# microsoft/ptgnn

Hardware: NVIDIA H100
Metric: edges/sec per GNN layer (higher is better)
Workload: dtype f32

## Files before the change

ptgnn_b200/csrc/fused_mp.cu:

```cuda
#include "fused_mp.cuh"

#include <cuda_bf16.h>
#include <cuda_fp16.h>
#include <float.h>
#include <stdlib.h>

#include <type_traits>

#include "tc_common.cuh"

namespace ptgnn {
namespace fused {

using tc::mbar_arrive;
using tc::mbar_init;
using tc::mbar_wait;

constexpr int NUM_THREADS = 12 * 32;
constexpr int GATHER_WARP0 = 8, GATHER_THREADS = 64;
constexpr int SCHED_WARP = 10;
constexpr int NUM_CONSUMER_WARPS = 8 + 2;
constexpr int NUM_SLOTS = 3, LOOKAHEAD = 2;
constexpr int SLOT_BYTES = 32768;
constexpr int RING_BYTES = NUM_SLOTS * SLOT_BYTES;
constexpr int META_RING = 8;
constexpr int SCHED_RING = 4;
constexpr int CONSUMER_REGS = 224, PRODUCER_REGS = 56;
static_assert(PRODUCER_REGS + 2 * CONSUMER_REGS <= 3 * 168, "register budgets exceed the launch allocation");
constexpr int NMAX = 64;
constexpr int ACC_PITCH = NMAX + 4;
constexpr int ACC_BYTES = kD * ACC_PITCH * 4;
constexpr int ALL_BAR_ID = 1, GRP_BAR_ID = 2;

struct Meta {
    int32_t tloff[128];
    uint32_t endmask[4];
    uint32_t lowmask[4];
    int32_t n, pad[3];
};
struct Sched {
    int32_t blk, pad[3];
    int32_t off[PTGNN_MAX_EDGE_TYPES + 4];
};
constexpr int ACC_OFF = RING_BYTES;
constexpr int AGG_OFF = RING_BYTES + ACC_BYTES;
__host__ __device__ constexpr int agg_bytes(int B) { return B * kD * 4; }
constexpr int SMEM_TAIL = META_RING * (int)sizeof(Meta) + SCHED_RING * (int)sizeof(Sched) + 256 ;
constexpr int smem_bytes(int B) { return 1024 + RING_BYTES + ACC_BYTES + agg_bytes(B) + SMEM_TAIL; }
static_assert(smem_bytes(kMaxBlockTargets) <= 232448, "shared memory budget");

struct Params {
    const unsigned char *src_rows, *tgt_rows;
    const uint4 *wpack;
    const int32_t *group_off, *src_f;
    const uint8_t *tl_f;
    const int32_t *row_ptr;
    void *out;
    int num_nodes, num_blocks, B, T, reduce, out_mode;
    int32_t *status;
    unsigned long long *trace;
    Epilogue epi;
};

__device__ __forceinline__ uint4 ldg_nc_u4(const uint4 *p) {
    uint4 r;
    asm volatile("ld.global.nc.L1::no_allocate.v4.u32 {%0,%1,%2,%3}, [%4];" : "=r"(r.x), "=r"(r.y), "=r"(r.z), "=r"(r.w) : "l"(p));
    return r;
}
__device__ __forceinline__ void named_bar_sync(int id, int threads) { asm volatile("bar.sync %0, %1;" ::"r"(id), "r"(threads) : "memory"); }
__device__ __forceinline__ uint32_t swz(int row, int q) { return (uint32_t)(row * 128 + ((q ^ (row & 7)) << 4)); }

constexpr int TRACE_ROLES = 3, TRACE_CAP = 8192;
__shared__ uint32_t trace_n[TRACE_ROLES];
__device__ __forceinline__ void trace_mark(const Params &p, int tag, uint32_t step) {
    if (p.trace == nullptr || blockIdx.x != 0) return;
    const int tid = (int)threadIdx.x;
    const int role = tid == GATHER_WARP0 * 32 ? 0 : (tid == 0 ? 1 : (tid == 128 ? 2 : -1));
    if (role < 0) return;
    const uint32_t n = trace_n[role];
    if (n >= TRACE_CAP) return;
    p.trace[role * TRACE_CAP + n] = ((unsigned long long)clock64() << 24) | ((unsigned long long)(step & 0xFFFFu) << 8) | (unsigned)(tag & 0xFF);
    trace_n[role] = n + 1;
}

struct Step { int blk, t, e, n, seg; bool first_sub, last_sub; };
template <int NSEG>
struct StepGen {
    const Sched *sched;
    uint64_t *sfull, *sempty;
    int T, nmax, lane;
    uint32_t it = 0;
    const Sched *tab = nullptr;
    int blk = -1, t = 0, e0 = 0, e = 0, e1 = 0, seg = 0;
    bool in_block = false;
    __device__ __forceinline__ int next(Step &s) {
        for (;;) {
            if (!in_block) {
                const uint32_t r = it % SCHED_RING;
                mbar_wait(&sfull[r], (it / SCHED_RING) & 1);
                tab = &sched[r];
                blk = tab->blk;
                if (blk < 0) return 2;
                in_block = true;
                t = -1; e = e1 = 0; seg = 0;
            }
            if (e < e1) {
                s.blk = blk; s.t = t; s.e = e; s.n = min(nmax, e1 - e); s.seg = seg;
                s.first_sub = e == e0; s.last_sub = e + nmax >= e1;
                if (++seg == NSEG) { seg = 0; e += nmax; }
                return 0;
            }
            ++t;
            while (t < T && tab->off[t + 1] == tab->off[t]) ++t;
            if (t >= T) {
                in_block = false;
                s.blk = blk;
                __syncwarp();
                if (lane == 0) mbar_arrive(&sempty[it % SCHED_RING]);
                ++it;
                return 1;
            }
            e0 = e = tab->off[t]; e1 = tab->off[t + 1]; seg = 0;
        }
    }
};

template <int RED>
__device__ __forceinline__ void continue_segment(float &t, float prev, float v, uint32_t start_bit) {
    if (RED == PTGNN_REDUCE_MAX)
        asm("{\n\t.reg .pred pc;\n\tsetp.eq.u32 pc, %3, 0;\n\t@pc max.f32 %0, %1, %2;\n\t}" : "+f"(t) : "f"(prev), "f"(v), "r"(start_bit));
    else if (RED == PTGNN_REDUCE_MIN)
        asm("{\n\t.reg .pred pc;\n\tsetp.eq.u32 pc, %3, 0;\n\t@pc min.f32 %0, %1, %2;\n\t}" : "+f"(t) : "f"(prev), "f"(v), "r"(start_bit));
    else
        asm("{\n\t.reg .pred pc;\n\tsetp.eq.u32 pc, %3, 0;\n\t@pc add.f32 %0, %1, %2;\n\t}" : "+f"(t) : "f"(prev), "f"(v), "r"(start_bit));
}
__device__ __forceinline__ void sts_f32_if(uint32_t addr, float v, uint32_t bit) {
    asm volatile("{\n\t.reg .pred pe;\n\tsetp.ne.u32 pe, %2, 0;\n\t@pe st.shared.f32 [%0], %1;\n\t}" ::"r"(addr), "f"(v), "r"(bit) : "memory");
}
__device__ __forceinline__ float4 lds_f32x4(uint32_t addr) {
    float4 v;
    asm volatile("ld.shared.v4.f32 {%0, %1, %2, %3}, [%4];" : "=f"(v.x), "=f"(v.y), "=f"(v.z), "=f"(v.w) : "r"(addr));
    return v;
}
__device__ __forceinline__ void sts_f32x4(uint32_t addr, float4 v) {
    asm volatile("st.shared.v4.f32 [%0], {%1, %2, %3, %4};" ::"r"(addr), "f"(v.x), "f"(v.y), "f"(v.z), "f"(v.w) : "memory");
}
__device__ __forceinline__ float lds_f32(uint32_t addr) {
    float v;
    asm volatile("ld.shared.f32 %0, [%1];" : "=f"(v) : "r"(addr) : "memory");
    return v;
}

__device__ __forceinline__ uint32_t pack_h2(__half a, __half b) {
    return (uint32_t)__half_as_ushort(a) | ((uint32_t)__half_as_ushort(b) << 16);
}
__device__ __forceinline__ bool split_f16(float x, __half &hi, __half &lo) {
    hi = __float2half_rn(x);
    lo = __float2half_rn((x - __half2float(hi)) * 2048.0f);
    return fabsf(x) < 65504.0f;
}

template <int RED> __device__ __forceinline__ float red_identity() {
    return RED == PTGNN_REDUCE_MAX ? -FLT_MAX : (RED == PTGNN_REDUCE_MIN ? FLT_MAX : 0.0f);
}
template <int RED> __device__ __forceinline__ float red_op(float a, float m) {
    if (RED == PTGNN_REDUCE_MAX) return fmaxf(a, m);
    if (RED == PTGNN_REDUCE_MIN) return fminf(a, m);
    return a + m;
}

template <int RED, bool WHOLE_ROW>
__device__ __forceinline__ void write_out_block(const Params *p, uint32_t agg_saddr, int row0, int row_lo, int row_hi, int r_first,
                                                int r_step, int q) {
    const float IDENT = red_identity<RED>();
    const int rows = min(p->B, p->num_nodes - row0);
    const int my_hi = min(row_hi, rows);
    const float4 ident4 = make_float4(IDENT, IDENT, IDENT, IDENT);
    auto finish_row = [&](auto mode_tag, auto plain_tag, int r, float4 a) {
        constexpr int MODE = decltype(mode_tag)::value;
        constexpr bool PLAIN = decltype(plain_tag)::value;
        const int v = row0 + r;
        if (!PLAIN) {
            if (RED == PTGNN_REDUCE_MEAN) {
                const int cnt = __ldg(p->row_ptr + v + 1) - __ldg(p->row_ptr + v);
                const float c = (float)(cnt < 1 ? 1 : cnt);
                a.x /= c; a.y /= c; a.z /= c; a.w /= c;
            }
            if (RED == PTGNN_REDUCE_MAX || RED == PTGNN_REDUCE_MIN) {
                if (a.x == IDENT) a.x = 0.0f;
                if (a.y == IDENT) a.y = 0.0f;
                if (a.z == IDENT) a.z = 0.0f;
                if (a.w == IDENT) a.w = 0.0f;
            }
            if (p->epi.act != PTGNN_ACT_NONE) {
                a.x = apply_act(a.x, p->epi.act); a.y = apply_act(a.y, p->epi.act);
                a.z = apply_act(a.z, p->epi.act); a.w = apply_act(a.w, p->epi.act);
            }
            if (WHOLE_ROW && p->epi.ln_w != nullptr) {
                float sum = (a.x + a.y) + (a.z + a.w);
#pragma unroll
                for (int o = 16; o > 0; o >>= 1) sum += __shfl_xor_sync(0xffffffffu, sum, o);
                const float mean = sum / (float)kD;
                const float dx = a.x - mean, dy = a.y - mean, dz = a.z - mean, dw = a.w - mean;
                float qq = (dx * dx + dy * dy) + (dz * dz + dw * dw);
#pragma unroll
                for (int o = 16; o > 0; o >>= 1) qq += __shfl_xor_sync(0xffffffffu, qq, o);
                const float rstd = rsqrtf(qq / (float)kD + p->epi.ln_eps);
                const float4 w = *reinterpret_cast<const float4 *>(p->epi.ln_w + q * 4);
                const float4 b = *reinterpret_cast<const float4 *>(p->epi.ln_b + q * 4);
                a.x = dx * rstd * w.x + b.x; a.y = dy * rstd * w.y + b.y;
                a.z = dz * rstd * w.z + b.z; a.w = dw * rstd * w.w + b.w;
            }
        }
        if (MODE == 1) {
            __nv_bfloat162 lo = __floats2bfloat162_rn(a.x, a.y), hi = __floats2bfloat162_rn(a.z, a.w);
            uint2 pk;
            pk.x = *reinterpret_cast<uint32_t *>(&lo); pk.y = *reinterpret_cast<uint32_t *>(&hi);
            reinterpret_cast<uint2 *>(p->out)[(size_t)v * (kD / 4) + q] = pk;
        } else if (MODE == 2) {
            const __half2 h01 = __floats2half2_rn(a.x, a.y), h23 = __floats2half2_rn(a.z, a.w);
            const float2 f01 = __half22float2(h01), f23 = __half22float2(h23);
            const __half2 l01 = __floats2half2_rn((a.x - f01.x) * 2048.0f, (a.y - f01.y) * 2048.0f);
            const __half2 l23 = __floats2half2_rn((a.z - f23.x) * 2048.0f, (a.w - f23.y) * 2048.0f);
            uint2 *row = reinterpret_cast<uint2 *>(p->out) + (size_t)v * (2 * kD / 4);
            row[q] = make_uint2(*reinterpret_cast<const uint32_t *>(&h01), *reinterpret_cast<const uint32_t *>(&h23));
            row[kD / 4 + q] = make_uint2(*reinterpret_cast<const uint32_t *>(&l01), *reinterpret_cast<const uint32_t *>(&l23));
            const float big = fmaxf(fmaxf(fabsf(a.x), fabsf(a.y)), fmaxf(fabsf(a.z), fabsf(a.w)));
            if (!(big < 65504.0f) && p->status != nullptr) *reinterpret_cast<volatile int32_t *>(p->status) = 1;
        } else {
            reinterpret_cast<float4 *>(p->out)[(size_t)v * (kD / 4) + q] = a;
        }
    };
    auto write_rows = [&](auto mode_tag, auto plain_tag) {
        for (int r0 = row_lo + r_first; r0 < my_hi; r0 += 2 * r_step) {
            float4 v4[2];
#pragma unroll
            for (int u = 0; u < 2; ++u) {
                const int r = r0 + r_step * u;
                if (r < my_hi) {
                    const uint32_t rowa = agg_saddr + (uint32_t)(r * kD + q * 4) * 4u;
                    v4[u] = lds_f32x4(rowa);
                    sts_f32x4(rowa, ident4);
                }
            }
#pragma unroll
            for (int u = 0; u < 2; ++u)
                if (r0 + r_step * u < my_hi) finish_row(mode_tag, plain_tag, r0 + r_step * u, v4[u]);
        }
    };
    const bool plain = RED == PTGNN_REDUCE_SUM && p->epi.act == PTGNN_ACT_NONE && p->epi.ln_w == nullptr;
    using std::integral_constant;
    if (p->out_mode == 2) { if (plain) write_rows(integral_constant<int, 2>{}, integral_constant<bool, true>{}); else write_rows(integral_constant<int, 2>{}, integral_constant<bool, false>{}); }
    else if (p->out_mode == 1) { if (plain) write_rows(integral_constant<int, 1>{}, integral_constant<bool, true>{}); else write_rows(integral_constant<int, 1>{}, integral_constant<bool, false>{}); }
    else { if (plain) write_rows(integral_constant<int, 0>{}, integral_constant<bool, true>{}); else write_rows(integral_constant<int, 0>{}, integral_constant<bool, false>{}); }
}

template <int NPROD, int K, int NSEG, int RED>
__global__ void __launch_bounds__(NUM_THREADS, 1) fused_aggregate_kernel(const __grid_constant__ Params p) {
    constexpr int NPART = NPROD == 3 ? 2 : 1;
    constexpr int ROW_BYTES = K * 2 * NPART;
    constexpr int KCH = K / 64;
    constexpr int NT = NPART * KCH;
    constexpr int TILE_BYTES = NMAX * 128;
    static_assert(NT * TILE_BYTES <= SLOT_BYTES, "slot size");
    constexpr bool BF16 = NPROD == 1;

    extern __shared__ unsigned char smem_raw[];
    unsigned char *ring = smem_raw + ((1024u - (smem_u32(smem_raw) & 1023u)) & 1023u);
    float *acc_s = reinterpret_cast<float *>(ring + ACC_OFF);
    float *agg_s = reinterpret_cast<float *>(ring + AGG_OFF);
    unsigned char *tail = ring + AGG_OFF + agg_bytes(p.B);
    Meta *meta_ring = reinterpret_cast<Meta *>(tail);
    Sched *sched = reinterpret_cast<Sched *>(tail + META_RING * sizeof(Meta));
    uint64_t *bars = reinterpret_cast<uint64_t *>(tail + META_RING * sizeof(Meta) + SCHED_RING * sizeof(Sched));
    uint64_t *x_full = bars, *x_empty = bars + 3, *sched_full = bars + 6, *sched_empty = bars + 10;

    const int warp = __shfl_sync(0xffffffffu, (int)(threadIdx.x >> 5), 0);
    const int lane = threadIdx.x & 31;
    if (threadIdx.x == 0) {
        for (int s = 0; s < NUM_SLOTS; ++s) { mbar_init(&x_full[s], 2 * GATHER_THREADS); mbar_init(&x_empty[s], 8); }
        for (int r = 0; r < SCHED_RING; ++r) { mbar_init(&sched_full[r], 1); mbar_init(&sched_empty[r], NUM_CONSUMER_WARPS); }
        for (int r = 0; r < TRACE_ROLES; ++r) trace_n[r] = 0;
        tc::mbar_init_fence();
    }
    __syncthreads();
    const int T = p.T;

    if (warp >= GATHER_WARP0) {
        tc::reg_dealloc<PRODUCER_REGS>();
        if (warp == SCHED_WARP) {
            for (uint32_t i = 0;; ++i) {
                const uint32_t r = i % SCHED_RING;
                mbar_wait(&sched_empty[r], ((i / SCHED_RING) & 1) ^ 1);
                const long long blk = (long long)blockIdx.x + (long long)i * gridDim.x;
                const bool valid = blk < p.num_blocks;
                Sched *e = &sched[r];
                if (valid) {
                    for (int t = lane; t <= T; t += 32) e->off[t] = __ldg(p.group_off + blk * T + t);
                }
                if (lane == 0) e->blk = valid ? (int)blk : -1;
                __syncwarp();
                if (lane == 0) mbar_arrive(&sched_full[r]);
                if (!valid) break;
            }
        } else if (warp < GATHER_WARP0 + GATHER_THREADS / 32) {
            const int g = (int)threadIdx.x - GATHER_WARP0 * 32;
            const int q = g & 7, rsub = g >> 3;
            StepGen<NSEG> gen{sched, sched_full, sched_empty, T, NMAX, lane};
            uint32_t c_issue = 0, c_done = 0, sgc = 0;
            Step cur, nxt;
            bool has_nxt = false;
            int idx_nxt[NMAX / 8];
            int tl_a[NMAX / 64], tl_b[NMAX / 64];
            auto fetch = [&]() {
                int ev;
                do { ev = gen.next(nxt); } while (ev == 1);
                has_nxt = ev == 0;
                if (!has_nxt) return;
                if (nxt.seg == 0) {
#pragma unroll
                    for (int i = 0; i < NMAX / 8; ++i) {
                        const int r = rsub + 8 * i;
                        idx_nxt[i] = r < nxt.n ? __ldg(p.src_f + nxt.e + r) : -1;
                    }
#pragma unroll
                    for (int half = 0; half < NMAX / 64; ++half) {
                        const int c = g + 64 * half;
                        tl_a[half] = c < nxt.n ? (int)__ldg(p.tl_f + nxt.e + c) : -1;
                        tl_b[half] = c + 1 < nxt.n ? (int)__ldg(p.tl_f + nxt.e + c + 1) : -2;
                    }
                } else {
#pragma unroll
                    for (int i = 0; i < NMAX / 8; ++i) {
                        const int r = rsub + 8 * i;
                        idx_nxt[i] = r < nxt.n ? nxt.blk * p.B + (int)__ldg(p.tl_f + nxt.e + r) : -1;
                    }
                }
            };
            auto finish_meta = [&](const Step &st) {
                if (st.seg != 0) return;
                Meta *m = &meta_ring[sgc % META_RING];
#pragma unroll
                for (int half = 0; half < NMAX / 64; ++half) {
                    const int c = g + 64 * half;
                    const bool valid = tl_a[half] >= 0;
                    const bool end = valid && tl_b[half] != tl_a[half];
                    m->tloff[c] = valid ? tl_a[half] * (kD * 4) : 0;
                    const uint32_t word = __ballot_sync(0xffffffffu, end);
                    const uint32_t low = __ballot_sync(0xffffffffu, valid && tl_a[half] < (p.B >> 1));
                    if (lane == 0) { m->endmask[c >> 5] = word; m->lowmask[c >> 5] = low; }
                }
                if (g == 0) m->n = st.n;
                ++sgc;
            };
            auto issue_next = [&]() {
                cur = nxt;
                int idx[NMAX / 8];
#pragma unroll
                for (int i = 0; i < NMAX / 8; ++i) idx[i] = idx_nxt[i];
                finish_meta(cur);
                const uint32_t slot = c_issue % NUM_SLOTS;
                trace_mark(p, 1, c_issue);
                mbar_wait(&x_empty[slot], ((c_issue / NUM_SLOTS) & 1) ^ 1);
                trace_mark(p, 2, c_issue);
                const unsigned char *rows = cur.seg == 0 ? p.src_rows : p.tgt_rows;
                const uint32_t sbase = smem_u32(ring + slot * SLOT_BYTES) + swz(rsub, q);
#pragma unroll
                for (int i = 0; i < NMAX / 8; ++i) {
                    if (idx[i] >= 0) {
                        const unsigned char *src = rows + (size_t)idx[i] * ROW_BYTES + q * 16;
#pragma unroll
                        for (int ti = 0; ti < NT; ++ti)
                            cp_async16(sbase + ti * TILE_BYTES + i * 1024, src + (ti / KCH) * (K * 2) + (ti % KCH) * 128, 16);
                    }
                }
                trace_mark(p, 3, c_issue);
                ++c_issue;
            };
            fetch();
            bool more = has_nxt;
            while (more) {
                const uint32_t slot = c_issue % NUM_SLOTS;
                issue_next();
                asm volatile("cp.async.mbarrier.arrive.noinc.shared::cta.b64 [%0];" ::"r"(smem_u32(&x_full[slot])) : "memory");
                trace_mark(p, 4, c_done);
                mbar_arrive(&x_full[slot]);
                ++c_done;
                fetch();
                more = has_nxt;
            }
            cp_async_wait<0>();
        }
    } else {
        tc::reg_alloc<CONSUMER_REGS>();
        constexpr bool SPLIT = NPROD == 3;
        const int eg = warp >> 2, ew = warp & 3;
        const int d = ew * 32 + lane;
        const int gq = lane >> 2, tq = lane & 3;
        const int f0 = 64 * eg + 16 * ew + gq;
        const int fw = SPLIT ? 64 * eg + (d & 63) : d, half = SPLIT ? d >> 6 : eg;
        const uint32_t aggcol_s = smem_u32(agg_s + fw);
        const uint32_t accrow_s = smem_u32(acc_s + fw * ACC_PITCH);
        const int grp_bar = GRP_BAR_ID + eg;
        const int stage_bar = SPLIT ? grp_bar : ALL_BAR_ID, stage_threads = SPLIT ? 128 : 256;
        const float IDENT = red_identity<RED>();
        StepGen<NSEG> gen{sched, sched_full, sched_empty, T, NMAX, lane};
        {
            const int row_lo = half == 0 ? 0 : (p.B >> 1), row_hi = half == 0 ? (p.B >> 1) : p.B;
            for (int r = row_lo; r < row_hi; ++r) agg_s[r * kD + fw] = IDENT;
        }
        uint32_t sg = 0, xs = 0;
        int w_t = -1, w_seg = -1;
        uint32_t wf[NPART][K / 16][4];
        float acc_m[32], acc_c[32];
        float acc = IDENT;
        auto load_weights = [&](const Step &st) {
            const uint32_t *wp = reinterpret_cast<const uint32_t *>(p.wpack + (size_t)(st.t * NSEG + st.seg) * NPART * (K / 8) * 128);
#pragma unroll
            for (int part = 0; part < NPART; ++part)
#pragma unroll
                for (int ks = 0; ks < K / 16; ++ks)
#pragma unroll
                    for (int i = 0; i < 4; ++i) {
                        const int c4 = (part * (K / 8) + 2 * ks + (i >> 1)), f = f0 + 8 * (i & 1);
                        wf[part][ks][i] = __ldg(wp + ((size_t)c4 * 128 + f) * 4 + tq);
                    }
            w_t = st.t; w_seg = st.seg;
            trace_mark(p, 11, xs);
        };
        auto mma = [&](auto nb_tag, uint32_t slot_addr) {
            constexpr int NB = decltype(nb_tag)::value;
#pragma unroll
            for (int ks = 0; ks < K / 16; ++ks) {
                const int kc = ks >> 2, kk = ks & 3;
                const uint64_t x_hi = tc::make_smem_desc_sw128(slot_addr + kc * TILE_BYTES) + kk * 2;
                const uint64_t x_lo = tc::make_smem_desc_sw128(slot_addr + (KCH + kc) * TILE_BYTES) + kk * 2;
                auto one = [&](float (&dacc)[32], const uint32_t (&a)[4], uint64_t desc) {
                    if (NB == 1) tc::wgmma_16_rs_n16<BF16>(dacc, a, desc);
                    else if (NB == 2) tc::wgmma_16_rs_n32<BF16>(dacc, a, desc);
                    else if (NB == 3) tc::wgmma_16_rs_n48<BF16>(dacc, a, desc);
                    else tc::wgmma_16_rs_n64<BF16>(dacc, a, desc);
                };
                one(acc_m, wf[0][ks], x_hi);
                if (NPROD == 3) {
                    one(acc_c, wf[0][ks], x_lo);
                    one(acc_c, wf[NPART - 1][ks], x_hi);
                }
            }
        };
        Step s, nx;
        int ev = gen.next(s);
        while (ev != 2) {
            if (ev == 0) {
                trace_mark(p, 10, xs);
                if (s.t != w_t || s.seg != w_seg) load_weights(s);
                const uint32_t slot = xs % NUM_SLOTS;
                mbar_wait(&x_full[slot], (xs / NUM_SLOTS) & 1);
                tc::fence_proxy_async_smem();
                trace_mark(p, 12, xs);
                if (tc::warp_uniform(s.seg) == 0) {
#pragma unroll
                    for (int i = 0; i < 32; ++i) { acc_m[i] = 0.0f; acc_c[i] = 0.0f; }
                }
                const uint32_t slot_addr = smem_u32(ring + slot * SLOT_BYTES);
                const int nb = tc::warp_uniform((s.n + 15) >> 4);
                tc::wgmma_fence();
                using std::integral_constant;
                if (nb == 1) mma(integral_constant<int, 1>{}, slot_addr);
                else if (nb == 2) mma(integral_constant<int, 2>{}, slot_addr);
                else if (nb == 3) mma(integral_constant<int, 3>{}, slot_addr);
                else mma(integral_constant<int, 4>{}, slot_addr);
                tc::wgmma_commit();
                trace_mark(p, 13, xs);
                tc::wgmma_wait<0>();
                tc::fence_acc(acc_m);
                tc::fence_acc(acc_c);
                __syncwarp();
                if (lane == 0) mbar_arrive(&x_empty[slot]);
                trace_mark(p, 14, xs);
                ++xs;
                const int evn = gen.next(nx);
                if (SPLIT && evn == 0 && (nx.t != w_t || nx.seg != w_seg)) load_weights(nx);
                if (s.seg == NSEG - 1) {
                    trace_mark(p, 20, sg);
                    named_bar_sync(stage_bar, stage_threads);
#pragma unroll
                    for (int j = 0; j < 8; ++j) {
                        if (8 * j < 16 * nb) {
#pragma unroll
                        for (int h = 0; h < 2; ++h) {
                            float v0 = acc_m[4 * j + 2 * h], v1 = acc_m[4 * j + 2 * h + 1];
                            if (NPROD == 3) { v0 = fmaf(acc_c[4 * j + 2 * h], 1.0f / 2048.0f, v0); v1 = fmaf(acc_c[4 * j + 2 * h + 1], 1.0f / 2048.0f, v1); }
                            *reinterpret_cast<float2 *>(acc_s + (f0 + 8 * h) * ACC_PITCH + 8 * j + 2 * tq) = make_float2(v0, v1);
                        }
                        }
                    }
                    named_bar_sync(stage_bar, stage_threads);
                    trace_mark(p, 21, sg);
                    const Meta *m = &meta_ring[sg % META_RING];
                    const int n = s.n;
                    int split = __popc(m->lowmask[0]) + __popc(m->lowmask[1]);
                    const int c_lo = half == 0 ? 0 : split, c_hi = half == 0 ? split : n;
                    constexpr int W = 16;
                    for (int c0 = c_lo & ~15; c0 < c_hi; c0 += 16) {
                        uint32_t vm[W];
#pragma unroll
                        for (int j = 0; j < W / 4; ++j) {
                            const float4 v4 = lds_f32x4(accrow_s + (uint32_t)(c0 + 4 * j) * 4u);
                            vm[4 * j] = __float_as_uint(v4.x); vm[4 * j + 1] = __float_as_uint(v4.y);
                            vm[4 * j + 2] = __float_as_uint(v4.z); vm[4 * j + 3] = __float_as_uint(v4.w);
                        }
                        uint32_t addr[W];
#pragma unroll
                        for (int j = 0; j < W / 4; ++j) {
                            const int4 o = *reinterpret_cast<const int4 *>(&m->tloff[c0 + 4 * j]);
                            addr[4 * j] = aggcol_s + o.x; addr[4 * j + 1] = aggcol_s + o.y;
                            addr[4 * j + 2] = aggcol_s + o.z; addr[4 * j + 3] = aggcol_s + o.w;
                        }
                        const uint32_t endw = (m->endmask[c0 >> 5] >> (c0 & 31)) & 0xFFFFu;
                        const uint32_t prev_end = c0 == 0 ? 1u : (m->endmask[(c0 - 1) >> 5] >> ((c0 - 1) & 31)) & 1u;
                        const uint32_t startw = (endw << 1) | prev_end;
                        const int first = c_lo > c0 ? c_lo - c0 : 0, last = c_hi - c0 < W ? c_hi - c0 : W;
                        const uint32_t storew = endw & (0xFFFFu << first) & (0xFFFFu >> (W - last));
                        float pre[W];
#pragma unroll
                        for (int c = 0; c < W; ++c) pre[c] = lds_f32(addr[c]);
                        float t[W];
                        constexpr bool ADD = RED == PTGNN_REDUCE_SUM || RED == PTGNN_REDUCE_MEAN;
#pragma unroll
                        for (int c = 0; c < W; ++c) {
                            float v = __uint_as_float(vm[c]);
                            if (NPROD == 1) {
                                v = __bfloat162float(__float2bfloat16_rn(v));
                                vm[c] = __float_as_uint(v);
                            }
                            t[c] = ADD ? __fadd_rn(pre[c], v) : red_op<RED>(pre[c], v);
                        }
                        continue_segment<RED>(t[0], acc, __uint_as_float(vm[0]), startw & 1u);
#pragma unroll
                        for (int c = 1; c < W; ++c) continue_segment<RED>(t[c], t[c - 1], __uint_as_float(vm[c]), startw & (1u << c));
                        acc = t[W - 1];
#pragma unroll
                        for (int c = 0; c < W; ++c) sts_f32_if(addr[c], t[c], storew & (1u << c));
                    }
                    trace_mark(p, 22, sg);
                    ++sg;
                }
                s = nx; ev = evn;
                continue;
            }
            const int blk = s.blk;
            const int evn = gen.next(nx);
            if (SPLIT && evn == 0 && (nx.t != w_t || nx.seg != w_seg)) load_weights(nx);
            trace_mark(p, 23, sg);
            if (SPLIT && p.epi.ln_w == nullptr) {
                named_bar_sync(grp_bar, 128);
                write_out_block<RED, false>(&p, smem_u32(agg_s), blk * p.B, 0, p.B, 2 * ew + (lane >> 4), 8, 16 * eg + (lane & 15));
            } else {
                const int wbar = SPLIT ? ALL_BAR_ID : grp_bar, wthreads = SPLIT ? 256 : 128;
                named_bar_sync(wbar, wthreads);
                const int row_lo = eg == 0 ? 0 : (p.B >> 1), row_hi = eg == 0 ? (p.B >> 1) : p.B;
                write_out_block<RED, true>(&p, smem_u32(agg_s), blk * p.B, row_lo, row_hi, ew, 4, lane);
                named_bar_sync(wbar, wthreads);
            }
            trace_mark(p, 24, sg);
            s = nx; ev = evn;
        }
    }
}

__global__ void __launch_bounds__(256) pack_states_kernel(const float *__restrict__ h, long long rows, int K,
                                                          uint4 *__restrict__ out, int32_t *__restrict__ status) {
    const long long total = rows * (K / 8);
    bool bad = false;
    for (long long i = (long long)blockIdx.x * blockDim.x + threadIdx.x; i < total; i += (long long)gridDim.x * blockDim.x) {
        const long long row = i / (K / 8);
        const int c8 = (int)(i - row * (K / 8));
        const float4 a = ld_stream_f4(reinterpret_cast<const float4 *>(h + row * K + c8 * 8));
        const float4 b = ld_stream_f4(reinterpret_cast<const float4 *>(h + row * K + c8 * 8 + 4));
        const float x[8] = {a.x, a.y, a.z, a.w, b.x, b.y, b.z, b.w};
        __half hi[8], lo[8];
#pragma unroll
        for (int j = 0; j < 8; ++j) bad |= !split_f16(x[j], hi[j], lo[j]);
        uint4 vh, vl;
        vh.x = pack_h2(hi[0], hi[1]); vh.y = pack_h2(hi[2], hi[3]); vh.z = pack_h2(hi[4], hi[5]); vh.w = pack_h2(hi[6], hi[7]);
        vl.x = pack_h2(lo[0], lo[1]); vl.y = pack_h2(lo[2], lo[3]); vl.z = pack_h2(lo[4], lo[5]); vl.w = pack_h2(lo[6], lo[7]);
        uint4 *dst = out + row * (K / 4);
        dst[c8] = vh;
        dst[K / 8 + c8] = vl;
    }
    if (bad && status != nullptr) *reinterpret_cast<volatile int32_t *>(status) = 1;
}

struct WeightSrc {
    const float *w[PTGNN_MAX_EDGE_TYPES];
};
template <int NPROD>
__global__ void __launch_bounds__(256) pack_weights_kernel(const __grid_constant__ WeightSrc src, int num_types, int K, int nseg,
                                                           uint4 *__restrict__ out, int32_t *__restrict__ status) {
    constexpr int NPART = NPROD == 3 ? 2 : 1;
    const int per_mat = nseg * (K / 8) * 128;
    const long long total = (long long)num_types * per_mat;
    bool bad = false;
    for (long long i = (long long)blockIdx.x * blockDim.x + threadIdx.x; i < total; i += (long long)gridDim.x * blockDim.x) {
        const int t = (int)(i / per_mat);
        int r = (int)(i - (long long)t * per_mat);
        const int seg = r / ((K / 8) * 128);
        r -= seg * (K / 8) * 128;
        const int c4 = r / 128, d = r % 128;
        const float *row = src.w[t] + (size_t)d * (nseg * K) + seg * K + c4 * 8;
        float x[8];
#pragma unroll
        for (int j = 0; j < 8; ++j) x[j] = row[j];
        const size_t base = ((size_t)(t * nseg + seg) * NPART) * (K / 8) * 128;
        if (NPROD == 3) {
            __half hi[8], lo[8];
#pragma unroll
            for (int j = 0; j < 8; ++j) bad |= !split_f16(x[j], hi[j], lo[j]);
            uint4 vh, vl;
            vh.x = pack_h2(hi[0], hi[1]); vh.y = pack_h2(hi[2], hi[3]); vh.z = pack_h2(hi[4], hi[5]); vh.w = pack_h2(hi[6], hi[7]);
            vl.x = pack_h2(lo[0], lo[1]); vl.y = pack_h2(lo[2], lo[3]); vl.z = pack_h2(lo[4], lo[5]); vl.w = pack_h2(lo[6], lo[7]);
            out[base + (size_t)c4 * 128 + d] = vh;
            out[base + (size_t)(K / 8 + c4) * 128 + d] = vl;
        } else {
            uint4 v;
            __nv_bfloat162 p0 = __floats2bfloat162_rn(x[0], x[1]), p1 = __floats2bfloat162_rn(x[2], x[3]);
            __nv_bfloat162 p2 = __floats2bfloat162_rn(x[4], x[5]), p3 = __floats2bfloat162_rn(x[6], x[7]);
            v.x = *reinterpret_cast<uint32_t *>(&p0); v.y = *reinterpret_cast<uint32_t *>(&p1);
            v.z = *reinterpret_cast<uint32_t *>(&p2); v.w = *reinterpret_cast<uint32_t *>(&p3);
            out[base + (size_t)c4 * 128 + d] = v;
        }
    }
    if (bad && status != nullptr) *reinterpret_cast<volatile int32_t *>(status + 1) = 1;
}

bool supported(int nprod, int K, int D, int use_target) {
    (void)use_target;
    if (D != kD) return false;
    if (nprod == 3) return K == 64 || K == 128;
    if (nprod == 1) return K == 64 || K == 128 || K == 256;
    return false;
}
size_t packed_weight_bytes(int nprod, int num_types, int K, int use_target) {
    const int nseg = use_target ? 2 : 1, npart = nprod == 3 ? 2 : 1;
    return ws_slice((size_t)num_types * nseg * npart * (K / 8) * 128, 16);
}
size_t packed_state_bytes(int nprod, int64_t rows, int K) {
    return nprod == 3 ? ws_slice((size_t)rows * K * 4 + 16, 1) : 0;
}
int recommended_block_targets(int64_t num_nodes) {
    if (num_nodes <= 0) return kMaxBlockTargets;
    const int64_t waves = ceil_div(num_nodes, (int64_t)kMaxBlockTargets * 132);
    int64_t B = ceil_div(num_nodes, waves * 132);
    B = (B + 7) / 8 * 8;
    if (B < 8) B = 8;
    if (B > kMaxBlockTargets) B = kMaxBlockTargets;
    return (int)B;
}

int pack_weights(int nprod, int num_types, int K, int use_target, const float *const *weights, void *packed, int32_t *status,
                 cudaStream_t st) {
    WeightSrc src{};
    for (int t = 0; t < num_types; ++t) src.w[t] = weights[t];
    const int nseg = use_target ? 2 : 1;
    {
        TimedScope timed__(PTGNN_KERNEL_PACK, st);
        if (nprod == 3) pack_weights_kernel<3><<<132, 256, 0, st>>>(src, num_types, K, nseg, static_cast<uint4 *>(packed), status);
        else pack_weights_kernel<1><<<132, 256, 0, st>>>(src, num_types, K, nseg, static_cast<uint4 *>(packed), status);
    }
    PTGNN_LAUNCHED();
    return PTGNN_OK;
}

int pack_states(const float *h, int64_t rows, int K, void *packed, int32_t *status, cudaStream_t st) {
    if (rows <= 0) return PTGNN_OK;
    const int64_t items = rows * (K / 8);
    const unsigned grid = (unsigned)(ceil_div(items, 256) < 132 * 8 ? ceil_div(items, 256) : 132 * 8);
    {
        TimedScope timed__(PTGNN_KERNEL_PACK, st);
        pack_states_kernel<<<grid, 256, 0, st>>>(h, (long long)rows, K, static_cast<uint4 *>(packed), status);
    }
    PTGNN_LAUNCHED();
    return PTGNN_OK;
}

template <int NPROD, int K, int NSEG, int RED>
static int launch_one(const Params &p, cudaStream_t st) {
    auto kernel = fused_aggregate_kernel<NPROD, K, NSEG, RED>;
    const int smem = smem_bytes(p.B);
    PTGNN_CUDA(cudaFuncSetAttribute(kernel, cudaFuncAttributeMaxDynamicSharedMemorySize, smem));
    const int sms = sm_count();
    const int grid = p.num_blocks < sms ? p.num_blocks : sms;
    {
        TimedScope timed__(PTGNN_KERNEL_MESSAGE, st);
        kernel<<<grid, NUM_THREADS, smem, st>>>(p);
    }
    PTGNN_LAUNCHED();
    return PTGNN_OK;
}
template <int NPROD, int K, int NSEG>
static int launch_red(const Params &p, cudaStream_t st) {
    switch (p.reduce) {
        case PTGNN_REDUCE_SUM: return launch_one<NPROD, K, NSEG, PTGNN_REDUCE_SUM>(p, st);
        case PTGNN_REDUCE_MEAN: return launch_one<NPROD, K, NSEG, PTGNN_REDUCE_MEAN>(p, st);
        case PTGNN_REDUCE_MAX: return launch_one<NPROD, K, NSEG, PTGNN_REDUCE_MAX>(p, st);
        default: return launch_one<NPROD, K, NSEG, PTGNN_REDUCE_MIN>(p, st);
    }
}
template <int NPROD, int K>
static int launch_seg(const Params &p, int use_target, cudaStream_t st) {
    return use_target ? launch_red<NPROD, K, 2>(p, st) : launch_red<NPROD, K, 1>(p, st);
}

static unsigned long long *g_trace_dev = nullptr;
static unsigned long long *trace_buffer() {
    static int want = -1;
    if (want < 0) { const char *e = getenv("PTGNN_FUSED_TRACE"); want = (e && e[0] == '1') ? 1 : 0; }
    if (!want) return nullptr;
    if (!g_trace_dev && cudaMalloc(&g_trace_dev, TRACE_ROLES * TRACE_CAP * 8) != cudaSuccess) return nullptr;
    cudaMemset(g_trace_dev, 0, TRACE_ROLES * TRACE_CAP * 8);
    return g_trace_dev;
}

int aggregate(const AggregateArgs &a, cudaStream_t st) {
    PTGNN_CHECK_ARG(supported(a.nprod, a.K, kD, a.use_target), "fused aggregate: unsupported nprod=%d K=%d", a.nprod, a.K);
    PTGNN_CHECK_ARG(a.block_targets >= 8 && a.block_targets <= kMaxBlockTargets, "fused aggregate: block_targets=%d out of [8, %d]",
                    a.block_targets, kMaxBlockTargets);
    PTGNN_CHECK_ARG(a.num_types > 0 && a.num_types <= PTGNN_MAX_EDGE_TYPES, "fused aggregate: bad num_types=%d", a.num_types);
    PTGNN_CHECK_ARG(a.reduce >= PTGNN_REDUCE_SUM && a.reduce <= PTGNN_REDUCE_MIN, "fused aggregate: bad reduce %d", a.reduce);
    if (a.num_nodes <= 0) return PTGNN_OK;
    PTGNN_CHECK_ARG(a.src_rows && a.group_off && a.packed_weights && a.out, "fused aggregate: null pointer");
    PTGNN_CHECK_ARG(!a.use_target || a.tgt_rows, "fused aggregate: null target rows");
    PTGNN_CHECK_ARG(a.reduce != PTGNN_REDUCE_MEAN || a.row_ptr, "fused aggregate: mean needs row_ptr");
    Params p{};
    p.src_rows = static_cast<const unsigned char *>(a.src_rows);
    p.tgt_rows = static_cast<const unsigned char *>(a.tgt_rows);
    p.wpack = static_cast<const uint4 *>(a.packed_weights);
    p.group_off = a.group_off; p.src_f = a.src_f; p.tl_f = a.tl_f; p.row_ptr = a.row_ptr;
    p.out = a.out; p.num_nodes = (int)a.num_nodes; p.B = a.block_targets;
    p.num_blocks = (int)ceil_div(a.num_nodes, a.block_targets);
    p.T = a.num_types; p.reduce = a.reduce; p.out_mode = a.out_mode; p.status = a.status; p.epi = a.epi;
    p.trace = trace_buffer();
#ifdef PTGNN_FUSED_QUICK
    return a.nprod == 3 ? launch_one<3, 128, 1, PTGNN_REDUCE_SUM>(p, st) : launch_one<1, 128, 1, PTGNN_REDUCE_SUM>(p, st);
#else
    if (a.nprod == 3) {
        if (a.K == 64) return launch_seg<3, 64>(p, a.use_target, st);
        return launch_seg<3, 128>(p, a.use_target, st);
    }
    if (a.K == 64) return launch_seg<1, 64>(p, a.use_target, st);
    if (a.K == 128) return launch_seg<1, 128>(p, a.use_target, st);
    return launch_seg<1, 256>(p, a.use_target, st);
#endif
}

}
}

extern "C" int ptgnn_b200_debug_fused_trace(unsigned long long *out) {
    using namespace ptgnn::fused;
    if (!g_trace_dev) return 0;
    if (out != nullptr) {
        cudaDeviceSynchronize();
        cudaMemcpy(out, g_trace_dev, TRACE_ROLES * TRACE_CAP * 8, cudaMemcpyDeviceToHost);
    }
    return TRACE_CAP;
}
```

Measured before the change: 1.208 billion.

## Offload segmented reduction and writeout to dedicated reducer warpgroup

Adds a fourth warpgroup of reducer warps that performs the segmented scatter-reduce into the aggregation tile and the output writeout. The MMA consumer warps now only stage accumulators into shared memory and signal through an acc_full/acc_empty mbarrier pair. This is meant to overlap the reduction with the next tile's wgmma instead of running them serially inside the consumer warps. In exchange, consumer register budgets drop from 224 to 184 and a single acc staging buffer makes consumers wait on the reducers. The low/high row split and the lowmask bookkeeping are removed.

Result: faster. 1.325 billion (median of 6 runs) (+9.7%).

```diff
diff --git a/ptgnn_b200/csrc/fused_mp.cu b/ptgnn_b200/csrc/fused_mp.cu
--- a/ptgnn_b200/csrc/fused_mp.cu
+++ b/ptgnn_b200/csrc/fused_mp.cu
@@ -16,26 +16,26 @@
 using tc::mbar_init;
 using tc::mbar_wait;
 
-constexpr int NUM_THREADS = 12 * 32;
+constexpr int NUM_THREADS = 16 * 32;
 constexpr int GATHER_WARP0 = 8, GATHER_THREADS = 64;
 constexpr int SCHED_WARP = 10;
-constexpr int NUM_CONSUMER_WARPS = 8 + 2;
+constexpr int REDUCER_WARP0 = 12;
+constexpr int SCHED_READER_WARPS = 8 + 2 + 4;
 constexpr int NUM_SLOTS = 3, LOOKAHEAD = 2;
 constexpr int SLOT_BYTES = 32768;
 constexpr int RING_BYTES = NUM_SLOTS * SLOT_BYTES;
 constexpr int META_RING = 8;
 constexpr int SCHED_RING = 4;
-constexpr int CONSUMER_REGS = 224, PRODUCER_REGS = 56;
-static_assert(PRODUCER_REGS + 2 * CONSUMER_REGS <= 3 * 168, "register budgets exceed the launch allocation");
+constexpr int PRODUCER_REGS = 56, CONSUMER_REGS = 184, REDUCER_REGS = 88;
+static_assert(PRODUCER_REGS + 2 * CONSUMER_REGS + REDUCER_REGS <= 4 * 128, "register budgets exceed the launch allocation");
 constexpr int NMAX = 64;
 constexpr int ACC_PITCH = NMAX + 4;
 constexpr int ACC_BYTES = kD * ACC_PITCH * 4;
-constexpr int ALL_BAR_ID = 1, GRP_BAR_ID = 2;
+constexpr int RED_BAR_ID = 1;
 
 struct Meta {
     int32_t tloff[128];
     uint32_t endmask[4];
-    uint32_t lowmask[4];
     int32_t n, pad[3];
 };
 struct Sched {
@@ -70,12 +70,12 @@
 __device__ __forceinline__ void named_bar_sync(int id, int threads) { asm volatile("bar.sync %0, %1;" ::"r"(id), "r"(threads) : "memory"); }
 __device__ __forceinline__ uint32_t swz(int row, int q) { return (uint32_t)(row * 128 + ((q ^ (row & 7)) << 4)); }
 
-constexpr int TRACE_ROLES = 3, TRACE_CAP = 8192;
+constexpr int TRACE_ROLES = 4, TRACE_CAP = 8192;
 __shared__ uint32_t trace_n[TRACE_ROLES];
 __device__ __forceinline__ void trace_mark(const Params &p, int tag, uint32_t step) {
     if (p.trace == nullptr || blockIdx.x != 0) return;
     const int tid = (int)threadIdx.x;
-    const int role = tid == GATHER_WARP0 * 32 ? 0 : (tid == 0 ? 1 : (tid == 128 ? 2 : -1));
+    const int role = tid == GATHER_WARP0 * 32 ? 0 : (tid == 0 ? 1 : (tid == 128 ? 2 : (tid == REDUCER_WARP0 * 32 ? 3 : -1)));
     if (role < 0) return;
     const uint32_t n = trace_n[role];
     if (n >= TRACE_CAP) return;
@@ -83,7 +83,7 @@
     trace_n[role] = n + 1;
 }
 
-struct Step { int blk, t, e, n, seg; bool first_sub, last_sub; };
+struct Step { int blk, t, e, n, seg; };
 template <int NSEG>
 struct StepGen {
     const Sched *sched;
@@ -91,36 +91,33 @@
     int T, nmax, lane;
     uint32_t it = 0;
     const Sched *tab = nullptr;
-    int blk = -1, t = 0, e0 = 0, e = 0, e1 = 0, seg = 0;
-    bool in_block = false;
+    int blk = -1, t = 0, e = 0, e1 = 0, seg = 0;
     __device__ __forceinline__ int next(Step &s) {
         for (;;) {
-            if (!in_block) {
+            if (tab == nullptr) {
                 const uint32_t r = it % SCHED_RING;
                 mbar_wait(&sfull[r], (it / SCHED_RING) & 1);
+                blk = sched[r].blk;
+                if (blk < 0) return 2;
                 tab = &sched[r];
-                blk = tab->blk;
-                if (blk < 0) return 2;
-                in_block = true;
                 t = -1; e = e1 = 0; seg = 0;
             }
             if (e < e1) {
                 s.blk = blk; s.t = t; s.e = e; s.n = min(nmax, e1 - e); s.seg = seg;
-                s.first_sub = e == e0; s.last_sub = e + nmax >= e1;
                 if (++seg == NSEG) { seg = 0; e += nmax; }
                 return 0;
             }
             ++t;
             while (t < T && tab->off[t + 1] == tab->off[t]) ++t;
             if (t >= T) {
-                in_block = false;
+                tab = nullptr;
                 s.blk = blk;
                 __syncwarp();
                 if (lane == 0) mbar_arrive(&sempty[it % SCHED_RING]);
                 ++it;
                 return 1;
             }
-            e0 = e = tab->off[t]; e1 = tab->off[t + 1]; seg = 0;
+            e = tab->off[t]; e1 = tab->off[t + 1]; seg = 0;
         }
     }
 };
@@ -169,12 +166,10 @@
     return a + m;
 }
 
-template <int RED, bool WHOLE_ROW>
-__device__ __forceinline__ void write_out_block(const Params *p, uint32_t agg_saddr, int row0, int row_lo, int row_hi, int r_first,
-                                                int r_step, int q) {
+template <int RED>
+__device__ __forceinline__ void write_out_block(const Params *p, uint32_t agg_saddr, int row0, int r_first, int r_step, int q) {
     const float IDENT = red_identity<RED>();
-    const int rows = min(p->B, p->num_nodes - row0);
-    const int my_hi = min(row_hi, rows);
+    const int my_hi = min(p->B, p->num_nodes - row0);
     const float4 ident4 = make_float4(IDENT, IDENT, IDENT, IDENT);
     auto finish_row = [&](auto mode_tag, auto plain_tag, int r, float4 a) {
         constexpr int MODE = decltype(mode_tag)::value;
@@ -196,7 +191,7 @@
                 a.x = apply_act(a.x, p->epi.act); a.y = apply_act(a.y, p->epi.act);
                 a.z = apply_act(a.z, p->epi.act); a.w = apply_act(a.w, p->epi.act);
             }
-            if (WHOLE_ROW && p->epi.ln_w != nullptr) {
+            if (p->epi.ln_w != nullptr) {
                 float sum = (a.x + a.y) + (a.z + a.w);
 #pragma unroll
                 for (int o = 16; o > 0; o >>= 1) sum += __shfl_xor_sync(0xffffffffu, sum, o);
@@ -232,7 +227,7 @@
         }
     };
     auto write_rows = [&](auto mode_tag, auto plain_tag) {
-        for (int r0 = row_lo + r_first; r0 < my_hi; r0 += 2 * r_step) {
+        for (int r0 = r_first; r0 < my_hi; r0 += 2 * r_step) {
             float4 v4[2];
 #pragma unroll
             for (int u = 0; u < 2; ++u) {
@@ -274,19 +269,89 @@
     Sched *sched = reinterpret_cast<Sched *>(tail + META_RING * sizeof(Meta));
     uint64_t *bars = reinterpret_cast<uint64_t *>(tail + META_RING * sizeof(Meta) + SCHED_RING * sizeof(Sched));
     uint64_t *x_full = bars, *x_empty = bars + 3, *sched_full = bars + 6, *sched_empty = bars + 10;
+    uint64_t *acc_full = bars + 14, *acc_empty = bars + 15;
 
     const int warp = __shfl_sync(0xffffffffu, (int)(threadIdx.x >> 5), 0);
     const int lane = threadIdx.x & 31;
     if (threadIdx.x == 0) {
         for (int s = 0; s < NUM_SLOTS; ++s) { mbar_init(&x_full[s], 2 * GATHER_THREADS); mbar_init(&x_empty[s], 8); }
-        for (int r = 0; r < SCHED_RING; ++r) { mbar_init(&sched_full[r], 1); mbar_init(&sched_empty[r], NUM_CONSUMER_WARPS); }
+        for (int r = 0; r < SCHED_RING; ++r) { mbar_init(&sched_full[r], 1); mbar_init(&sched_empty[r], SCHED_READER_WARPS); }
+        mbar_init(acc_full, 8);
+        mbar_init(acc_empty, 4);
         for (int r = 0; r < TRACE_ROLES; ++r) trace_n[r] = 0;
         tc::mbar_init_fence();
     }
     __syncthreads();
     const int T = p.T;
 
-    if (warp >= GATHER_WARP0) {
+    if (warp >= REDUCER_WARP0) {
+        tc::reg_dealloc<REDUCER_REGS>();
+        const int d = (int)threadIdx.x - REDUCER_WARP0 * 32, rw = warp - REDUCER_WARP0;
+        const uint32_t aggcol_s = smem_u32(agg_s + d);
+        const uint32_t accrow_s = smem_u32(acc_s + d * ACC_PITCH);
+        const float IDENT = red_identity<RED>();
+        for (int r = 0; r < p.B; ++r) agg_s[r * kD + d] = IDENT;
+        StepGen<NSEG> gen{sched, sched_full, sched_empty, T, NMAX, lane};
+        uint32_t sg = 0;
+        float acc = IDENT;
+        Step s;
+        for (int ev; (ev = gen.next(s)) != 2;) {
+            if (ev == 1) {
+                trace_mark(p, 33, sg);
+                named_bar_sync(RED_BAR_ID, 128);
+                write_out_block<RED>(&p, smem_u32(agg_s), s.blk * p.B, rw, 4, lane);
+                named_bar_sync(RED_BAR_ID, 128);
+                trace_mark(p, 34, sg);
+                continue;
+            }
+            if (s.seg != NSEG - 1) continue;
+            trace_mark(p, 30, sg);
+            mbar_wait(acc_full, sg & 1);
+            trace_mark(p, 31, sg);
+            const Meta *m = &meta_ring[sg % META_RING];
+            const int n = s.n;
+            constexpr int W = 16;
+            for (int c0 = 0; c0 < n; c0 += W) {
+                uint32_t vm[W];
+#pragma unroll
+                for (int j = 0; j < W / 4; ++j) {
+                    const float4 v4 = lds_f32x4(accrow_s + (uint32_t)(c0 + 4 * j) * 4u);
+                    vm[4 * j] = __float_as_uint(v4.x); vm[4 * j + 1] = __float_as_uint(v4.y);
+                    vm[4 * j + 2] = __float_as_uint(v4.z); vm[4 * j + 3] = __float_as_uint(v4.w);
+                }
+                uint32_t addr[W];
+#pragma unroll
+                for (int j = 0; j < W / 4; ++j) {
+                    const int4 o = *reinterpret_cast<const int4 *>(&m->tloff[c0 + 4 * j]);
+                    addr[4 * j] = aggcol_s + o.x; addr[4 * j + 1] = aggcol_s + o.y;
+                    addr[4 * j + 2] = aggcol_s + o.z; addr[4 * j + 3] = aggcol_s + o.w;
+                }
+                const uint32_t endw = (m->endmask[c0 >> 5] >> (c0 & 31)) & 0xFFFFu;
+                const uint32_t prev_end = c0 == 0 ? 1u : (m->endmask[(c0 - 1) >> 5] >> ((c0 - 1) & 31)) & 1u;
+                const uint32_t startw = (endw << 1) | prev_end;
+                float pre[W];
+#pragma unroll
+                for (int c = 0; c < W; ++c) pre[c] = lds_f32(addr[c]);
+                float t[W];
+                constexpr bool ADD = RED == PTGNN_REDUCE_SUM || RED == PTGNN_REDUCE_MEAN;
+#pragma unroll
+                for (int c = 0; c < W; ++c) {
+                    const float v = __uint_as_float(vm[c]);
+                    t[c] = ADD ? __fadd_rn(pre[c], v) : red_op<RED>(pre[c], v);
+                }
+                continue_segment<RED>(t[0], acc, __uint_as_float(vm[0]), startw & 1u);
+#pragma unroll
+                for (int c = 1; c < W; ++c) continue_segment<RED>(t[c], t[c - 1], __uint_as_float(vm[c]), startw & (1u << c));
+                acc = t[W - 1];
+#pragma unroll
+                for (int c = 0; c < W; ++c) sts_f32_if(addr[c], t[c], endw & (1u << c));
+            }
+            __syncwarp();
+            if (lane == 0) mbar_arrive(acc_empty);
+            trace_mark(p, 32, sg);
+            ++sg;
+        }
+    } else if (warp >= GATHER_WARP0) {
         tc::reg_dealloc<PRODUCER_REGS>();
         if (warp == SCHED_WARP) {
             for (uint32_t i = 0;; ++i) {
@@ -347,8 +412,7 @@
                     const bool end = valid && tl_b[half] != tl_a[half];
                     m->tloff[c] = valid ? tl_a[half] * (kD * 4) : 0;
                     const uint32_t word = __ballot_sync(0xffffffffu, end);
-                    const uint32_t low = __ballot_sync(0xffffffffu, valid && tl_a[half] < (p.B >> 1));
-                    if (lane == 0) { m->endmask[c >> 5] = word; m->lowmask[c >> 5] = low; }
+                    if (lane == 0) m->endmask[c >> 5] = word;
                 }
                 if (g == 0) m->n = st.n;
                 ++sgc;
@@ -393,27 +457,14 @@
         }
     } else {
         tc::reg_alloc<CONSUMER_REGS>();
-        constexpr bool SPLIT = NPROD == 3;
         const int eg = warp >> 2, ew = warp & 3;
-        const int d = ew * 32 + lane;
         const int gq = lane >> 2, tq = lane & 3;
         const int f0 = 64 * eg + 16 * ew + gq;
-        const int fw = SPLIT ? 64 * eg + (d & 63) : d, half = SPLIT ? d >> 6 : eg;
-        const uint32_t aggcol_s = smem_u32(agg_s + fw);
-        const uint32_t accrow_s = smem_u32(acc_s + fw * ACC_PITCH);
-        const int grp_bar = GRP_BAR_ID + eg;
-        const int stage_bar = SPLIT ? grp_bar : ALL_BAR_ID, stage_threads = SPLIT ? 128 : 256;
-        const float IDENT = red_identity<RED>();
         StepGen<NSEG> gen{sched, sched_full, sched_empty, T, NMAX, lane};
-        {
-            const int row_lo = half == 0 ? 0 : (p.B >> 1), row_hi = half == 0 ? (p.B >> 1) : p.B;
-            for (int r = row_lo; r < row_hi; ++r) agg_s[r * kD + fw] = IDENT;
-        }
         uint32_t sg = 0, xs = 0;
         int w_t = -1, w_seg = -1;
         uint32_t wf[NPART][K / 16][4];
         float acc_m[32], acc_c[32];
-        float acc = IDENT;
         auto load_weights = [&](const Step &st) {
             const uint32_t *wp = reinterpret_cast<const uint32_t *>(p.wpack + (size_t)(st.t * NSEG + st.seg) * NPART * (K / 8) * 128);
 #pragma unroll
@@ -474,97 +525,41 @@
                 trace_mark(p, 13, xs);
                 tc::wgmma_wait<0>();
                 tc::fence_acc(acc_m);
-                tc::fence_acc(acc_c);
+                if (NPROD == 3) tc::fence_acc(acc_c);
                 __syncwarp();
                 if (lane == 0) mbar_arrive(&x_empty[slot]);
                 trace_mark(p, 14, xs);
                 ++xs;
                 const int evn = gen.next(nx);
-                if (SPLIT && evn == 0 && (nx.t != w_t || nx.seg != w_seg)) load_weights(nx);
+                if (evn == 0 && (nx.t != w_t || nx.seg != w_seg)) load_weights(nx);
                 if (s.seg == NSEG - 1) {
                     trace_mark(p, 20, sg);
-                    named_bar_sync(stage_bar, stage_threads);
+                    mbar_wait(acc_empty, (sg & 1) ^ 1);
+                    trace_mark(p, 21, sg);
 #pragma unroll
                     for (int j = 0; j < 8; ++j) {
                         if (8 * j < 16 * nb) {
 #pragma unroll
                         for (int h = 0; h < 2; ++h) {
                             float v0 = acc_m[4 * j + 2 * h], v1 = acc_m[4 * j + 2 * h + 1];
-                            if (NPROD == 3) { v0 = fmaf(acc_c[4 * j + 2 * h], 1.0f / 2048.0f, v0); v1 = fmaf(acc_c[4 * j + 2 * h + 1], 1.0f / 2048.0f, v1); }
+                            if (NPROD == 3) {
+                                v0 = fmaf(acc_c[4 * j + 2 * h], 1.0f / 2048.0f, v0); v1 = fmaf(acc_c[4 * j + 2 * h + 1], 1.0f / 2048.0f, v1);
+                            } else {
+                                v0 = __bfloat162float(__float2bfloat16_rn(v0)); v1 = __bfloat162float(__float2bfloat16_rn(v1));
+                            }
                             *reinterpret_cast<float2 *>(acc_s + (f0 + 8 * h) * ACC_PITCH + 8 * j + 2 * tq) = make_float2(v0, v1);
                         }
                         }
                     }
-                    named_bar_sync(stage_bar, stage_threads);
-                    trace_mark(p, 21, sg);
-                    const Meta *m = &meta_ring[sg % META_RING];
-                    const int n = s.n;
-                    int split = __popc(m->lowmask[0]) + __popc(m->lowmask[1]);
-                    const int c_lo = half == 0 ? 0 : split, c_hi = half == 0 ? split : n;
-                    constexpr int W = 16;
-                    for (int c0 = c_lo & ~15; c0 < c_hi; c0 += 16) {
-                        uint32_t vm[W];
-#pragma unroll
-                        for (int j = 0; j < W / 4; ++j) {
-                            const float4 v4 = lds_f32x4(accrow_s + (uint32_t)(c0 + 4 * j) * 4u);
-                            vm[4 * j] = __float_as_uint(v4.x); vm[4 * j + 1] = __float_as_uint(v4.y);
-                            vm[4 * j + 2] = __float_as_uint(v4.z); vm[4 * j + 3] = __float_as_uint(v4.w);
-                        }
-                        uint32_t addr[W];
-#pragma unroll
-                        for (int j = 0; j < W / 4; ++j) {
-                            const int4 o = *reinterpret_cast<const int4 *>(&m->tloff[c0 + 4 * j]);
-                            addr[4 * j] = aggcol_s + o.x; addr[4 * j + 1] = aggcol_s + o.y;
-                            addr[4 * j + 2] = aggcol_s + o.z; addr[4 * j + 3] = aggcol_s + o.w;
-                        }
-                        const uint32_t endw = (m->endmask[c0 >> 5] >> (c0 & 31)) & 0xFFFFu;
-                        const uint32_t prev_end = c0 == 0 ? 1u : (m->endmask[(c0 - 1) >> 5] >> ((c0 - 1) & 31)) & 1u;
-                        const uint32_t startw = (endw << 1) | prev_end;
-                        const int first = c_lo > c0 ? c_lo - c0 : 0, last = c_hi - c0 < W ? c_hi - c0 : W;
-                        const uint32_t storew = endw & (0xFFFFu << first) & (0xFFFFu >> (W - last));
-                        float pre[W];
-#pragma unroll
-                        for (int c = 0; c < W; ++c) pre[c] = lds_f32(addr[c]);
-                        float t[W];
-                        constexpr bool ADD = RED == PTGNN_REDUCE_SUM || RED == PTGNN_REDUCE_MEAN;
-#pragma unroll
-                        for (int c = 0; c < W; ++c) {
-                            float v = __uint_as_float(vm[c]);
-                            if (NPROD == 1) {
-                                v = __bfloat162float(__float2bfloat16_rn(v));
-                                vm[c] = __float_as_uint(v);
-                            }
-                            t[c] = ADD ? __fadd_rn(pre[c], v) : red_op<RED>(pre[c], v);
-                        }
-                        continue_segment<RED>(t[0], acc, __uint_as_float(vm[0]), startw & 1u);
-#pragma unroll
-                        for (int c = 1; c < W; ++c) continue_segment<RED>(t[c], t[c - 1], __uint_as_float(vm[c]), startw & (1u << c));
-                        acc = t[W - 1];
-#pragma unroll
-                        for (int c = 0; c < W; ++c) sts_f32_if(addr[c], t[c], storew & (1u << c));
-                    }
+                    __syncwarp();
+                    if (lane == 0) mbar_arrive(acc_full);
                     trace_mark(p, 22, sg);
                     ++sg;
                 }
                 s = nx; ev = evn;
                 continue;
             }
-            const int blk = s.blk;
-            const int evn = gen.next(nx);
-            if (SPLIT && evn == 0 && (nx.t != w_t || nx.seg != w_seg)) load_weights(nx);
-            trace_mark(p, 23, sg);
-            if (SPLIT && p.epi.ln_w == nullptr) {
-                named_bar_sync(grp_bar, 128);
-                write_out_block<RED, false>(&p, smem_u32(agg_s), blk * p.B, 0, p.B, 2 * ew + (lane >> 4), 8, 16 * eg + (lane & 15));
-            } else {
-                const int wbar = SPLIT ? ALL_BAR_ID : grp_bar, wthreads = SPLIT ? 256 : 128;
-                named_bar_sync(wbar, wthreads);
-                const int row_lo = eg == 0 ? 0 : (p.B >> 1), row_hi = eg == 0 ? (p.B >> 1) : p.B;
-                write_out_block<RED, true>(&p, smem_u32(agg_s), blk * p.B, row_lo, row_hi, ew, 4, lane);
-                named_bar_sync(wbar, wthreads);
-            }
-            trace_mark(p, 24, sg);
-            s = nx; ev = evn;
+            ev = gen.next(s);
         }
     }
 }
```
